# CWNE88/topdogspectrumanalyser

Hardware: AMD Instinct MI355X
Metric: PSD frames/sec at 16384-pt FFT on synthetic 20 Msps IQ (higher is better)
Workload: dtype f32; 1 GPU

## Files before the change

topdogspectrumanalyser_amd/csrc/tdsa_capi_plan.cpp:

```cpp
#include "tdsa_capi_internal.hpp"

#include <cstdarg>

using namespace tdsa;

namespace tdsa {

static thread_local char g_err[512] = "ok";

int fail(int code, const char* fmt, ...) {
  va_list ap;
  va_start(ap, fmt);
  vsnprintf(g_err, sizeof(g_err), fmt, ap);
  va_end(ap);
  return code;
}

int join_streams(tdsa_plan p) {
  if (p->aux_busy) {
    for (int i = 0; i < p->n_overlap - 1; ++i) {
      HIPCHK(hipEventRecord(p->ev_aux[i], p->aux[i]));
      HIPCHK(hipStreamWaitEvent(p->stream, p->ev_aux[i], 0));
    }
    p->aux_busy = false;
// ... 74 lines not shown
  if (!native && !chirp)
    return fail(TDSA_ERR_ARG, "nfft=%d: need a power of two in [%d, %d] or any size in [2, %d]", nfft, 1 << kMinLog2N,
                1 << kBigMaxLog2N, kChirpMaxN);
  const bool big = native && nfft > (1 << kMaxLog2N);
  if (max_frames < 1) return fail(TDSA_ERR_ARG, "max_frames=%d must be >= 1", max_frames);
  int ndev = 0;
  HIPCHK(hipGetDeviceCount(&ndev));
  if (device_id < 0 || device_id >= ndev) return fail(TDSA_ERR_ARG, "device %d of %d", device_id, ndev);
  HIPCHK(hipSetDevice(device_id));
  tdsa_plan p = new (std::nothrow) tdsa_plan_s();
  if (!p) return fail(TDSA_ERR_NOMEM, "host allocation failed");
  p->device = device_id;
  p->nfft = nfft;
  p->log2n = ilog2i(nfft);
  p->max_frames = max_frames;
  p->big = big;
  p->chirp = chirp;
  if (chirp) {
    int m = 1 << kMinLog2N;
    if (nfft > (1 << 19)) {
      p->chirp_split = (nfft + 1) / 2;
      m = 1 << kBigMaxLog2N;
    } else {
      while (m < 2 * nfft - 1) m <<= 1;
    }
    p->m_fft = m;
    p->log2m = ilog2i(m);
    p->chirp_big = p->log2m > kMaxLog2N;
    p->log2n = p->chirp_big ? kMaxLog2N : p->log2m;
  }
  const int rc_init = plan_init(p);
  if (rc_init != TDSA_OK) {
    (void)tdsa_destroy(p);
    return rc_init;
  }
  *out = p;
  return TDSA_OK;
}

static int plan_init(tdsa_plan p) {
  const int device_id = p->device, nfft = p->nfft, max_frames = p->max_frames;
  const bool big = p->big;
  hipDeviceProp_t prop;
  HIPCHK(hipGetDeviceProperties(&prop, device_id));
  p->num_cu = prop.multiProcessorCount > 0 ? prop.multiProcessorCount : 256;
  p->avg_wg_min = nfft <= 4096 ? 48 : 128;
  HIPCHK(hipStreamCreateWithFlags(&p->stream, hipStreamNonBlocking));
  HIPCHK(hipEventCreate(&p->ev0));
  HIPCHK(hipEventCreate(&p->ev1));
  HIPCHK(hipEventCreateWithFlags(&p->ev_state, hipEventDisableTiming));
  const size_t nb = size_t(nfft) * sizeof(float);
  for (int f = 0; f < 3; ++f) HIPCHK(hipMalloc(&p->d_window[f], nb));
  if (!p->big && !p->chirp && p->log2n >= 11)
    for (int f = 0; f < 3; ++f) HIPCHK(hipMalloc(&p->d_window_perm[f], nb));
  const int tw_n = p->chirp ? (p->chirp_big ? (1 << kMaxLog2N) : p->m_fft) : nfft;
  HIPCHK(hipMalloc(&p->d_hold_max, nb));
  HIPCHK(hipMalloc(&p->d_hold_min, nb));
  HIPCHK(hipMalloc(&p->d_avg, size_t(nfft) * sizeof(double)));
  HIPCHK(hipMalloc(&p->d_dc_state, sizeof(float2)));
  HIPCHK(hipMalloc(&p->d_sums, (size_t(max_frames) + 8) * sizeof(float2)));
  HIPCHK(hipMalloc(&p->d_dc_sub, size_t(max_frames) * sizeof(float2)));
  HIPCHK(hipMalloc(&p->d_tare_base, nb));
  HIPCHK(hipMalloc(&p->d_tare_acc, nb));
  HIPCHK(hipMalloc(&p->d_trace_in, nb));
  HIPCHK(hipMalloc(&p->d_trace_live, nb));
  HIPCHK(hipMemsetAsync(p->d_dc_state, 0, sizeof(float2), p->stream));
  HIPCHK(hipMemsetAsync(p->d_avg, 0, size_t(nfft) * sizeof(double), p->stream));
  TRY(upload(unit_circle(tw_n), &p->d_tw));
  if (p->chirp) TRY(chirp_plan_init(p));
  if (big) {
    HIPCHK(hipMalloc(&p->d_sum, size_t(nfft) * sizeof(double)));
    HIPCHK(hipMalloc(&p->d_lin64, size_t(nfft) * sizeof(double)));
    {
      const int n1 = nfft >> 14;
      int split = p->num_cu / n1 > 1 ? p->num_cu / n1 : 1;
      const int gmax = p->max_frames < p->big_group ? p->max_frames : p->big_group;
      if (split > gmax) split = gmax;
      HIPCHK(hipMalloc(&p->d_acc, size_t(n1) * split * (size_t(1) << 14) * sizeof(float)));
    }
    const int nrow = 1 << kMaxLog2N;
    TRY(upload(seed_table(nfft, p->log2n), &p->d_tw_seed));
    TRY(upload(unit_circle(nrow), &p->d_tw_row));
    TRY(upload(std::vector<float>(nrow, 1.0f), &p->d_ones));
  }
  TRY(reset_hold(p, true, true));
  p->mode.db_mode = TDSA_DB_MAG;
  p->mode.power_scale = 1.0f;
  p->mode.log_floor = 1e-12f;
  p->mode.avg_mode = TDSA_AVG_OFF;
  p->mode.avg_n = 1;
  p->mode.dc_alpha = 1.0f;
  p->mode.cal_offset_db = 0.0f;
  p->mode.hold_flags = 0;
  HIPCHK(hipStreamSynchronize(p->stream));
  return TDSA_OK;
}

int tdsa_destroy(tdsa_plan p) {
  if (!p) return TDSA_OK;
  (void)hipSetDevice(p->device);
  for (hipStream_t a : p->aux)
    if (a) (void)hipStreamSynchronize(a);
  if (p->stream) (void)hipStreamSynchronize(p->stream);
  free_all({p->d_window[0], p->d_window[1], p->d_window[2], p->d_window_perm[0], p->d_window_perm[1],
                  p->d_window_perm[2], p->d_tw, p->d_hold_max, p->d_hold_min,
                  p->d_avg, p->d_lin, p->d_carry, p->d_agg, p->d_agg_w, p->d_chunk_a, p->d_chunk_v, p->d_cplx, p->d_real, p->d_lin1, p->d_db1, p->d_dc_state, p->d_sums, p->d_dc_sub,
                  p->d_tare_base, p->d_tare_acc, p->d_in_stage, p->d_out_stage, p->d_trace_in,
// ... 9 lines not shown
  for (hipEvent_t e : p->prof_events) (void)hipEventDestroy(e);
  if (p->ev0) (void)hipEventDestroy(p->ev0);
  if (p->ev1) (void)hipEventDestroy(p->ev1);
  if (p->ev_state) (void)hipEventDestroy(p->ev_state);
  for (hipEvent_t e : p->ev_aux)
    if (e) (void)hipEventDestroy(e);
  for (hipStream_t a : p->aux)
    if (a) (void)hipStreamDestroy(a);
  if (p->stream) (void)hipStreamDestroy(p->stream);
  delete p;
  return TDSA_OK;
}

int tdsa_get_info(tdsa_plan p, tdsa_info* out) {
  if (!p || !out) return fail(TDSA_ERR_ARG, "null argument");
  LaunchGeom g = p->big ? spectrum_geometry(kMaxLog2N, (p->nfft >> kMaxLog2N) * (p->max_frames < p->big_group ? p->max_frames : p->big_group), p->num_cu)
                        : spectrum_geometry(p->log2n, p->max_frames, p->num_cu);
  out->nfft = p->nfft;
  out->max_frames = p->max_frames;
  out->device_id = p->device;
  out->grid = g.grid;
  out->block = g.block;
  out->frames_per_block = g.fpw;
  out->lds_bytes = int(g.lds_bytes);
  out->num_cu = p->num_cu;
  out->frames_held_max = p->held_max;
  out->frames_held_min = p->held_min;
  out->avg_count = p->avg_count;
  out->version = TDSA_VERSION;
  return TDSA_OK;
}

static void big_window_model(tdsa_plan p, const float* w, const float scale[3]) {
  bool flat = true;
  for (int i = 1; i < p->nfft && flat; ++i) flat = w[i] == w[0];
  for (int f = 0; f < 3; ++f) {
    p->big_win[f] = BigWindow{flat ? 2 : 0, p->d_window[f], w[0] * scale[f]};
  }
}

int tdsa_set_window(tdsa_plan p, const float* w_host, int n) {
  if (!p || !w_host) return fail(TDSA_ERR_ARG, "null argument");
  if (n != p->nfft) return fail(TDSA_ERR_ARG, "window length %d != nfft %d", n, p->nfft);
  HIPCHK(hipSetDevice(p->device));
  JOIN(p);
  float scale[3];
  for (int f = 0; f < 3; ++f) scale[f] = in_format_consts(f).scale;
  std::vector<float> tmp(n);
  HIPCHK(hipStreamSynchronize(p->stream));
  for (int f = 0; f < 3; ++f) {
    for (int i = 0; i < n; ++i) tmp[i] = w_host[i] * scale[f];
    HIPCHK(hipMemcpy(p->d_window[f], tmp.data(), size_t(n) * sizeof(float), hipMemcpyHostToDevice));
    if (p->d_window_perm[f]) HIPCHK(launch_window_perm(p->log2n, p->d_window[f], p->d_window_perm[f], p->stream));
  }
  if (p->big) big_window_model(p, w_host, scale);
  if (p->chirp && p->log2m >= 10) {
    std::vector<float2> aw(n);
    std::vector<double> ca(n), sa(n);
    for (int i = 0; i < n; ++i) {
      const long long q = ((long long)i * i) % (2ll * n);
      const double ang = -M_PI * double(q) / double(n);
      ca[i] = std::cos(ang);
      sa[i] = std::sin(ang);
    }
    for (int f = 0; f < 3; ++f) {
      for (int i = 0; i < n; ++i) {
        const double wv = double(w_host[i]) * double(scale[f]);
        aw[i] = float2{float(wv * ca[i]), float(wv * sa[i])};
      }
      if (!p->d_chirp_aw[f]) HIPCHK(hipMalloc(&p->d_chirp_aw[f], aw.size() * sizeof(float2)));
      HIPCHK(hipMemcpy(p->d_chirp_aw[f], aw.data(), aw.size() * sizeof(float2), hipMemcpyHostToDevice));
    }
  }
  p->window_set = true;
  return TDSA_OK;
}

int tdsa_set_mode(tdsa_plan p, const tdsa_mode* m) {
  if (!p || !m) return fail(TDSA_ERR_ARG, "null argument");
  if (m->db_mode != TDSA_DB_MAG && m->db_mode != TDSA_DB_POW) return fail(TDSA_ERR_ARG, "db_mode %d", m->db_mode);
  if (m->avg_mode < TDSA_AVG_OFF || m->avg_mode > TDSA_AVG_LIN) return fail(TDSA_ERR_ARG, "avg_mode %d", m->avg_mode);
  if (m->dc_alpha > 1.0f) return fail(TDSA_ERR_ARG, "dc_alpha %g > 1", double(m->dc_alpha));
  if (!(m->log_floor >= 0.0f)) return fail(TDSA_ERR_ARG, "log_floor must be >= 0");
  tdsa_mode nm = *m;
  if (nm.avg_n < 1) nm.avg_n = 1;
  const bool avg_changed = nm.avg_mode != p->mode.avg_mode || nm.avg_n != p->mode.avg_n;
  p->mode = nm;
  if (avg_changed) p->avg_count = 0;
  return TDSA_OK;
}

int tdsa_set_overlap(tdsa_plan p, int n_streams) {
  if (!p) return fail(TDSA_ERR_ARG, "null plan");
  if (n_streams < 1 || n_streams > tdsa_plan_s::kMaxOverlap)
    return fail(TDSA_ERR_ARG, "n_streams=%d outside [1, %d]", n_streams, tdsa_plan_s::kMaxOverlap);
  HIPCHK(hipSetDevice(p->device));
  JOIN(p);
  for (int i = 0; i < n_streams - 1; ++i) {
    if (!p->aux[i]) {
      HIPCHK(hipStreamCreateWithFlags(&p->aux[i], hipStreamNonBlocking));
      HIPCHK(hipEventCreateWithFlags(&p->ev_aux[i], hipEventDisableTiming));
    }
  }
  p->n_overlap = n_streams;
  p->rr = 0;
  return TDSA_OK;
// ... 132 lines not shown
```

topdogspectrumanalyser_amd/csrc/tdsa_kernels.hpp:

```cpp
#pragma once
#include <hip/hip_runtime.h>
#include <stddef.h>
#include <stdint.h>

#include <atomic>

namespace tdsa {

inline hipError_t ensure_dynamic_lds(const void* fn, int bytes, std::atomic<unsigned long long>& done) {
  int dev = 0;
  hipError_t e = hipGetDevice(&dev);
  if (e != hipSuccess) return e;
  const unsigned long long bit = 1ull << (dev & 63);
  if (done.load(std::memory_order_acquire) & bit) return hipSuccess;
  e = hipFuncSetAttribute(fn, hipFuncAttributeMaxDynamicSharedMemorySize, bytes);
  if (e == hipSuccess) done.fetch_or(bit, std::memory_order_release);
  return e;
}

constexpr int kMinLog2N = 6;
constexpr int kMaxLog2N = 14;

constexpr int DC_NONE = 0, DC_FRAME_MEAN = 1, DC_TRACKED = 2;

// ... 8 lines not shown
  float* out_db;
  float* out_lin;
  float2* out_cplx;
  const float2* out_mul;
  int out_mul_rows;
  int in_valid;
  int out_valid;
  const float2* dc_sub;
  float2* dc_state;
  float* part_max;
  float* part_min;
  const float* tare;
  unsigned xor_mask;
  float in_off;
  float in_scale;
  int dc_mode;
  int db_mode;
  float pscale;
  float log_floor;
  float cal_db;
  int hold_flags;
  unsigned long long* dbg;
  const float* agg_w;
  float* agg_out;
  int agg_only;
  unsigned seg_magic;
  unsigned seg_frames;
  long long seg_in_stride;
  long long seg_out_stride;
  const void* pre_raw;
  long long pre_stride;
  const float2* pre_aw;
  int pre_c64;
  unsigned pre_xor;
  float pre_off;
  int post_n;
  float post_inv_m;
  int rows_twice;
  void* stats_part;
  unsigned band_lohi;
};
constexpr int kStatsRecBytes = 16;
inline int spectrum_waves_per_frame(int log2n) { return log2n <= 10 ? 1 : (1 << log2n) / 1024; }

struct LaunchGeom {
  int grid, block, fpw;
  size_t lds_bytes;
};

LaunchGeom spectrum_geometry(int log2n, int n_frames, int num_cu);
hipError_t launch_spectrum(int log2n, int in_c64, const SpecParams& p, const LaunchGeom& g,
                           hipStream_t s);
hipError_t launch_window_perm(int log2n, const float* w, float* w_perm, hipStream_t s);

__host__ __device__ inline void spectrum_unit_range(unsigned b, unsigned n_units, unsigned grid, int& u0, int& u1) {
  const unsigned upw = n_units / grid, urem = n_units - upw * grid;
  u0 = int(b * upw + b * urem / grid);
  u1 = int((b + 1) * upw + (b + 1) * urem / grid);
}

struct AvgParams {
  const float* lin;
  int n_frames, n;
  double* state;
  int count_in;
  int mode, avg_n;
  float log_floor, cal_db;
  const float* tare;
  float* out_db;
  float* state_max;
  float* state_min;
  int first_frame_index;
  int wg_chunks;
  int wg_fold;
  int wg_fpw;
  const float* agg;
  const double* chunk_a;
  const float* chunk_v;
  const float* agg_w_local;
  int state_only;
};
constexpr int kAvgMaxWgChunks = 1024;
__host__ __device__ inline void avg_wg_range(const AvgParams& p, int b, int& f0, int& f1) {
  const int fpw = p.wg_fpw > 1 ? p.wg_fpw : 1;
  int u0, u1;
  spectrum_unit_range(unsigned(b), unsigned((p.n_frames + fpw - 1) / fpw), unsigned(p.wg_chunks), u0, u1);
  f0 = u0 * fpw < p.n_frames ? u0 * fpw : p.n_frames;
  f1 = u1 * fpw < p.n_frames ? u1 * fpw : p.n_frames;
}
hipError_t launch_avg_scan(const AvgParams& p, hipStream_t s, double* carry);
int avg_scan_chunks(int n_frames);
hipError_t launch_avg_weights(const AvgParams& p, float* w, double* chunk_a, float* chunk_v, hipStream_t s);

hipError_t launch_frame_sums(const void* in, int in_c64, unsigned xor_mask, long long frame_stride,
                             int n, int n_frames, float2* sums, hipStream_t s);
hipError_t launch_dc_track(const float2* sums, int n, int n_frames, float alpha, float in_off,
                           float in_scale, float2* dc_state, float2* dc_sub, hipStream_t s, int parts = 1);

struct TraceParams {
  const float* db_in;
  int n;
  float cal_db;
  float* tare_acc;
  int tare_collect;
  int tare_first;
  int tare_finish;
// ... 151 lines not shown
```

topdogspectrumanalyser_amd/csrc/tdsa_spectrum.hip:

```cpp
#include "tdsa_kernels.hpp"

namespace tdsa {
template <int LOG2N> hipError_t launch_size(int in_c64, const SpecParams& p, const LaunchGeom& g, hipStream_t s);
template <int LOG2N> LaunchGeom geom_size(int n_frames, int num_cu);
template <int LOG2N> hipError_t perm_size(const float* w, float* wp, hipStream_t s);

#define TDSA_FOR_SIZES(X) X(6) X(7) X(8) X(9) X(10) X(11) X(12) X(13) X(14)
#define TDSA_DECL(k)                                                                                  \
  template <> hipError_t launch_size<k>(int, const SpecParams&, const LaunchGeom&, hipStream_t);      \
  template <> LaunchGeom geom_size<k>(int, int);                                                      \
  template <> hipError_t perm_size<k>(const float*, float*, hipStream_t);
TDSA_FOR_SIZES(TDSA_DECL)

LaunchGeom spectrum_geometry(int log2n, int n_frames, int num_cu) {
  switch (log2n) {
#define TDSA_CASE(k) case k: return geom_size<k>(n_frames, num_cu);
    TDSA_FOR_SIZES(TDSA_CASE)
#undef TDSA_CASE
    default: return LaunchGeom{1, 256, 1, 0};
  }
}

hipError_t launch_window_perm(int log2n, const float* w, float* wp, hipStream_t s) {
  switch (log2n) {
#define TDSA_CASE(k) case k: return perm_size<k>(w, wp, s);
    TDSA_FOR_SIZES(TDSA_CASE)
#undef TDSA_CASE
    default: return hipErrorInvalidValue;
  }
}

hipError_t launch_spectrum(int log2n, int in_c64, const SpecParams& p, const LaunchGeom& g, hipStream_t s) {
  switch (log2n) {
#define TDSA_CASE(k) case k: return launch_size<k>(in_c64, p, g, s);
    TDSA_FOR_SIZES(TDSA_CASE)
#undef TDSA_CASE
    default: return hipErrorInvalidValue;
  }
}
}
```

topdogspectrumanalyser_amd/csrc/tdsa_spectrum_c3_inst.hip:

```cpp
#include "tdsa_spectrum_kernel.hpp"

namespace tdsa {
hipError_t launch_c3_slide(const SpecParams& p, const LaunchGeom& g, hipStream_t s) {
  return (p.hold_flags & 1) ? launch_one<14, false, 16 | 1>(p, g, s) : launch_one<14, false, 16>(p, g, s);
}
}
```

topdogspectrumanalyser_amd/csrc/tdsa_spectrum_kernel.hpp:

```cpp
#pragma once
#ifndef TDSA_DEV
#undef TDSA_TIMELINE
#undef TDSA_DYN_PRIO
#endif
#include "tdsa_fft.hpp"
#include "tdsa_kernels.hpp"
#include "tdsa_wave.hpp"

namespace tdsa {

template <int LOG2N>
struct Cfg {
  static constexpr int N = 1 << LOG2N;
  static constexpr int SG = N / 32;
  static constexpr int TPF = 2 * SG;
  static constexpr int NPASS = (N >= 2048) ? 3 : 2;
  static constexpr int A = (NPASS == 3) ? N / 1024 : N / 32;
  static constexpr int M = 32 / A;
  static constexpr int H = A / 2;
  static constexpr bool INL = (M >= 8) && (NPASS == 3);
  static constexpr int R1 = INL ? A : H;
  static constexpr int CPT = INL ? M / 2 : M;
  static constexpr int WGT = TPF > 256 ? TPF : 256;
  static constexpr int FPW = WGT / TPF;
// ... 58 lines not shown
      constexpr int i = decltype(ic)::value;
      const u32x4 q = __builtin_amdgcn_raw_buffer_load_b128(r, voff, soff + 16 * i, 0);
      dst[4 * i] = q.x; dst[4 * i + 1] = q.y; dst[4 * i + 2] = q.z; dst[4 * i + 3] = q.w;
    });
  }
}

constexpr int kRowStorePolicy = 2;
constexpr float k10Log10_2 = 3.01029995663981195214f;
constexpr float kMagExactBelow = 1e-8f;

#define TDSA_SYNC()                                                        \
  do {                                                                     \
    if constexpr (C::TPF <= 64) {                                          \
      __builtin_amdgcn_fence(__ATOMIC_RELEASE, "wavefront");               \
      __builtin_amdgcn_wave_barrier();                                     \
      __builtin_amdgcn_fence(__ATOMIC_ACQUIRE, "wavefront");               \
    } else {                                                               \
      __syncthreads();                                                     \
    }                                                                      \
  } while (0)

#ifdef TDSA_DYN_PRIO
#define TDSA_PRIO(n) __builtin_amdgcn_s_setprio(n)
#else
#define TDSA_PRIO(n) do { } while (0)
#endif

#ifdef TDSA_TIMELINE
#define TDSA_STAMP(i)                                                                              \
  do {                                                                                             \
    if (p.dbg != nullptr && blockIdx.x == 0 && (tid & 63) == 0 && unit - u0 < 8)                   \
      tl[((unit - u0) * 16 + wave) * 16 + (i)] = __builtin_amdgcn_s_memtime();                      \
  } while (0)
#else
#define TDSA_STAMP(i)
#endif

typedef float lds_v2 __attribute__((ext_vector_type(2)));
typedef __attribute__((address_space(3))) volatile lds_v2* lds_vptr;
__device__ __forceinline__ c32 lds_ld(const c32* p) {
  const lds_v2 x = *(lds_vptr)(p);
  return c32{x.x, x.y};
}
__device__ __forceinline__ void lds_st(c32* p, c32 v) { *(lds_vptr)(p) = lds_v2{v.x, v.y}; }

__device__ __forceinline__ void swap_halves(c32& a, c32& b) {
  auto rx = __builtin_amdgcn_permlane32_swap(__float_as_uint(a.x), __float_as_uint(b.x), false, false);
  auto ry = __builtin_amdgcn_permlane32_swap(__float_as_uint(a.y), __float_as_uint(b.y), false, false);
  a.x = __uint_as_float(rx[0]); b.x = __uint_as_float(rx[1]);
  a.y = __uint_as_float(ry[0]); b.y = __uint_as_float(ry[1]);
}

template <int R, int BASE, int TOT>
__device__ __forceinline__ void radix(c32 (&v)[TOT]) {
  dit<R, BASE, TOT>(v);
}

__device__ __forceinline__ void combine(c32& e, c32& o, c32 w) {
  const float x1 = fmaf(w.x, o.x, fmaf(-w.y, o.y, e.x));
  const float y1 = fmaf(w.x, o.y, fmaf(w.y, o.x, e.y));
  o = c32{fmaf(2.0f, e.x, -x1), fmaf(2.0f, e.y, -y1)};
  e = c32{x1, y1};
}
template <int U, bool EXACT = false>
__device__ __forceinline__ void combine32(c32& e, c32& o, bool odd_half) {
  const c32 orot = c32{odd_half ? o.y : o.x, odd_half ? -o.x : o.y};
  o = orot;
  bf_w<U, 32, EXACT>(e, o);
}
template <int K, int R, bool EXACT = false>
__device__ __forceinline__ void combine_const(c32& e, c32& o) {
  bf_w<K, R, EXACT>(e, o);
}

template <int LOG2N, bool IN_C64, int HOLDX, int CHIRP = 0>
__global__ void __launch_bounds__(Cfg<LOG2N>::WGT, 4) spectrum_kernel(const SpecParams p) {
  constexpr int HOLD = HOLDX & 7;
  constexpr bool STATS = (HOLDX & 8) != 0;
  constexpr bool SLIDE = (HOLDX & 16) != 0;
  using C = Cfg<LOG2N>;
  constexpr int N = C::N, SG = C::SG, A = C::A, M = C::M, H = C::H, FPW = C::FPW, NPAD = C::NPAD;
  constexpr int LH = ilog2(H);
  constexpr bool INL = C::INL;
  constexpr int R1 = C::R1;
  constexpr int LR1 = ilog2(R1);
  constexpr int CPT = C::CPT;
  constexpr int DW = (CPT >= 2) ? CPT / 2 : 1;
  constexpr int NRAW = IN_C64 ? 1 : R1 * DW;
  constexpr int ROWB = (N / A) * 2;
  constexpr int RSTEP = INL ? 1 : 2;

  extern __shared__ __attribute__((aligned(16))) unsigned char smem[];
  c32* lds = reinterpret_cast<c32*>(smem);
  c32* twm = reinterpret_cast<c32*>(smem + C::DATA_BYTES);
  double* red = reinterpret_cast<double*>(smem + C::DATA_BYTES + size_t(C::TWM) * sizeof(c32));
#ifdef TDSA_TIMELINE
  unsigned long long* tl = reinterpret_cast<unsigned long long*>(smem + C::LDS_BYTES);
#endif

  const int tid = threadIdx.x;
  const int wave = tid >> 6;
#ifdef TDSA_TIMELINE
  const unsigned long long tl_entry = __builtin_amdgcn_s_memtime();
#endif
  const int h = (tid >> 5) & 1;
  const int g = wave * 32 + (tid & 31);
  constexpr bool UNI = C::TPF >= 64;
  const int slot = (FPW == 1) ? 0 : (UNI ? __builtin_amdgcn_readfirstlane(g / SG) : g / SG);
  const int t = (FPW == 1) ? g : g - slot * SG;
  c32* buf = lds + slot * NPAD;

  const int n_units = (p.n_frames + FPW - 1) / FPW;
  const unsigned upw = unsigned(n_units) / gridDim.x, urem = unsigned(n_units) - upw * gridDim.x;
  int u0 = int(blockIdx.x * upw + blockIdx.x * urem / gridDim.x);
  int u1 = int((blockIdx.x + 1) * upw + (blockIdx.x + 1) * urem / gridDim.x);
  auto frame_of = [&](int unit) -> int {
    if constexpr (HOLD == 4 && FPW > 1) return u0 * FPW + slot * (u1 - u0) + (unit - u0);
    else return unit * FPW + slot;
  };
  constexpr unsigned SB = IN_C64 ? 8u : 2u;
  const rsrc_t win_rsrc = make_rsrc(C::WIN_LDS ? p.window : p.window_perm, N * 4u);
  float* win_lds = reinterpret_cast<float*>(smem + C::LDS_BYTES - C::WIN_BYTES);
  constexpr bool TWF_LDS = C::TWF_BYTES != 0 && HOLD == 3 && !IN_C64;
  c32* twf_tab = reinterpret_cast<c32*>(smem + C::LDS_BYTES - C::WIN_BYTES - C::TWF_BYTES);
  if constexpr (TWF_LDS) {
    if (slot == 0) {
      if (h == 0) static_for<0, 3>([&](auto ic) { constexpr int j = decltype(ic)::value; twf_tab[j * SG + t] = p.tw[t * 2 * (j + 1)]; });
      static_for<0, 4>([&](auto ic) { constexpr int a = decltype(ic)::value; twf_tab[3 * SG + a * C::TPF + h * SG + t] = p.tw[t * (8 * a + h)]; });
    }
  }
  if constexpr (C::WIN_LDS) {
    for (int i = tid; i < N; i += C::WGT) win_lds[i] = p.window[i];
    __syncthreads();
  }
  const unsigned win_voff = (unsigned(h) * SG + unsigned(t)) * 16u;
  const bool odd_half = h != 0;
  constexpr bool AGG = HOLD == 4;
  float agg[AGG ? 16 : 1];
  static_for<0, (AGG ? 16 : 1)>([&](auto ic) { agg[decltype(ic)::value] = 0.f; });
  float hmax[(HOLD & 1) ? 16 : 1], hmin[(HOLD & 2) ? 16 : 1];
  static_for<0, 16>([&](auto ic) {
    constexpr int i = decltype(ic)::value;
    if constexpr ((HOLD & 1) != 0) hmax[i] = -INFINITY;
// ... 60 lines not shown
  };
  auto out_elem_off = [&](int frame) -> long long {
    const unsigned sgm = __umulhi(unsigned(frame), p.seg_magic);
    const unsigned fi = unsigned(frame) - sgm * p.seg_frames;
    return (long long)sgm * p.seg_out_stride + (long long)fi * N;
  };

  float win[16];
  auto load_window = [&] {
    if constexpr (CHIRP != 0) {
    } else if constexpr (C::WIN_LDS) {
      static_for<0, R1>([&](auto ic) {
        constexpr int i = decltype(ic)::value;
        static_for<0, CPT>([&](auto jc) {
          constexpr int jj = decltype(jc)::value;
          if constexpr (INL) win[jj * R1 + i] = win_lds[i * (N / A) + t * M + h * CPT + jj];
          else win[jj * R1 + i] = win_lds[(2 * i + h) * (N / A) + t * M + jj];
        });
      });
    } else {
      uint32_t wq[16];
      static_for<0, 4>([&](auto qc) { constexpr int q = decltype(qc)::value; buf_load<4>(win_rsrc, win_voff, q * (2u * SG * 16u), &wq[4 * q]); });
      static_for<0, 16>([&](auto ic) { constexpr int i = decltype(ic)::value; win[i] = __uint_as_float(wq[i]); });
    }
  };
  uint32_t raw[NRAW];
  auto load_frame_raw = [&](int frame) {
    if constexpr (!IN_C64) {
      const bool act = frame < p.n_frames;
      const unsigned char* fb = static_cast<const unsigned char*>(p.in) + in_byte_off(frame);
      if constexpr (UNI) {
        const rsrc_t r = make_rsrc(fb, (FPW == 1 || act) ? N * 2u : 0u);
        static_for<0, R1>([&](auto ic) {
          constexpr int i = decltype(ic)::value;
          if constexpr (M == 1) raw[i] = unsigned(__builtin_amdgcn_raw_buffer_load_b16(r, lane_in_off, RSTEP * i * ROWB, 0));
          else buf_load<DW>(r, lane_in_off, RSTEP * i * ROWB, &raw[i * DW]);
        });
      } else {
        static_for<0, R1>([&](auto ic) {
          constexpr int i = decltype(ic)::value;
          const unsigned char* row = fb + RSTEP * i * ROWB + lane_in_off;
          if (act) {
            if constexpr (M == 1) raw[i] = *reinterpret_cast<const uint16_t*>(row);
            else load_raw<DW>(row, &raw[i * DW]);
          } else {
            static_for<0, DW>([&](auto jc) { raw[i * DW + decltype(jc)::value] = 0u; });
          }
        });
      }
    }
  };
  if (u0 < u1) load_frame_raw(frame_of(u0));
  bool slide_full = true;
  unsigned slide_sum = 0;
  typedef unsigned short slide_u16x2 __attribute__((ext_vector_type(2)));
  static_assert(!SLIDE || (LOG2N == 14 && !IN_C64 && HOLD < 2 && !STATS && CHIRP == 0 && FPW == 1 && !INL && M == 2 && NRAW == 8),
                "sliding front end: the 16384-point byte-format dB-row instantiations, hold off / max hold");
  c32 twf_lo[3], twf_hi[4];
  constexpr bool TWF_RELOAD = (CHIRP == 3 || CHIRP == 4) && (LOG2N == 11 || LOG2N == 14);
  if constexpr (!TWF_LDS && !TWF_RELOAD) {
    static_for<0, 3>([&](auto ic) { constexpr int j = decltype(ic)::value; twf_lo[j] = p.tw[t * 2 * (j + 1)]; });
    static_for<0, 4>([&](auto ic) { constexpr int a = decltype(ic)::value; twf_hi[a] = p.tw[t * (8 * a + h)]; });
  }
  if constexpr (C::NPASS == 3) {
    if (tid < C::TWM) {
      const int b = tid / A, ka = tid % A;
      twm[tid] = p.tw[ka * b * (N / (32 * A))];
    }
  }
  if constexpr (!C::WIN_LDS) load_window();

#ifdef TDSA_TIMELINE
  if (p.dbg != nullptr && blockIdx.x == 0 && (tid & 63) == 0) {
    tl[(2 * 16 + wave) * 16 + 12] = tl_entry;
    tl[(2 * 16 + wave) * 16 + 13] = __builtin_amdgcn_s_memtime();
  }
#endif
  for (int unit = u0; unit < u1; ++unit) {
    const int frame = frame_of(unit);
    const bool active = frame < p.n_frames;
    TDSA_STAMP(0);

    c32 v[16];
    float sub_re = p.in_off, sub_im = p.in_off;
    float res_re = 0.f, res_im = 0.f;
    if constexpr (IN_C64) {
      if constexpr (CHIRP == 1 || CHIRP == 3) {
        static_assert(HOLD == 0 && UNI, "fused chirp transforms: complex64 instantiation without hold, whole waves per frame");
        {
          const unsigned char* rb = static_cast<const unsigned char*>(p.pre_raw) + (long long)frame * p.pre_stride;
          const unsigned nv = active ? unsigned(p.in_valid) : 0u;
          const rsrc_t ar = make_rsrc(p.pre_aw, nv * 8u);
          float dcx = 0.f, dcy = 0.f;
          if (active && p.dc_sub != nullptr) { const float2 d = p.dc_sub[frame]; dcx = d.x; dcy = d.y; }
          const unsigned xm = p.pre_xor & 0xffffu;
          if (p.pre_c64) {
            const rsrc_t rr = make_rsrc(rb, nv * 8u);
            static_for<0, 16>([&](auto ic) {
              constexpr int idx = decltype(ic)::value;
              constexpr int jj = idx / R1, i = idx % R1;
              const u32x2 q = __builtin_amdgcn_raw_buffer_load_b64(rr, lane_in_off + jj * 8u, RSTEP * i * (N / A) * 8, 0);
              const u32x2 w = __builtin_amdgcn_raw_buffer_load_b64(ar, lane_in_off + jj * 8u, RSTEP * i * (N / A) * 8, 0);
              v[idx] = cmul(c32{__uint_as_float(q.x) - dcx, __uint_as_float(q.y) - dcy}, c32{__uint_as_float(w.x), __uint_as_float(w.y)});
            });
          } else {
            const rsrc_t rr = make_rsrc(rb, nv * 2u);
            const unsigned roff = lane_in_off >> 2;
            static_for<0, 16>([&](auto ic) {
              constexpr int idx = decltype(ic)::value;
              constexpr int jj = idx / R1, i = idx % R1;
              const unsigned u = unsigned(__builtin_amdgcn_raw_buffer_load_b16(rr, roff + jj * 2u, RSTEP * i * (N / A) * 2, 0)) ^ xm;
              const u32x2 w = __builtin_amdgcn_raw_buffer_load_b64(ar, lane_in_off + jj * 8u, RSTEP * i * (N / A) * 8, 0);
              v[idx] = cmul(c32{(float(u & 0xffu) - p.pre_off) - dcx, (float((u >> 8) & 0xffu) - p.pre_off) - dcy},
                            c32{__uint_as_float(w.x), __uint_as_float(w.y)});
            });
          }
        }
      } else {
      const unsigned char* fb = static_cast<const unsigned char*>(p.in) + in_byte_off(frame);
      static_for<0, 16>([&](auto ic) {
        constexpr int idx = decltype(ic)::value;
        constexpr int jj = idx / R1, i = idx % R1;
        const c32* row = reinterpret_cast<const c32*>(fb + RSTEP * i * (N / A) * 8 + lane_in_off);
// ... 570 lines not shown
```

topdogspectrumanalyser_amd/csrc/tdsa_spectrum_passes.inc:

```
    if constexpr (!IN_C64 && SG >= 32) {
      int* redi = reinterpret_cast<int*>(red);
      unsigned slide_ti = 0, slide_tq = 0;
      if constexpr (SLIDE) {
        if (slide_full) {
          unsigned li = 0, lq = 0;
          static_for<0, NRAW / 2>([&](auto ic) {
            constexpr int i = decltype(ic)::value;
            raw[i] ^= xm_v;
            li = __builtin_amdgcn_udot4(raw[i], 0x00010001u, li, false);
            lq = __builtin_amdgcn_udot4(raw[i], 0x01000100u, lq, false);
          });
          slide_sum = li | (lq << 16);
        }
        static_for<NRAW / 2, NRAW>([&](auto ic) {
          constexpr int i = decltype(ic)::value;
          raw[i] ^= xm_v;
          slide_ti = __builtin_amdgcn_udot4(raw[i], 0x00010001u, slide_ti, false);
          slide_tq = __builtin_amdgcn_udot4(raw[i], 0x01000100u, slide_tq, false);
        });
        const unsigned up = slide_ti | (slide_tq << 16);
        slide_ti = __builtin_amdgcn_udot2(__builtin_bit_cast(slide_u16x2, slide_sum), __builtin_bit_cast(slide_u16x2, 0x00000001u), slide_ti, false);
        slide_tq = __builtin_amdgcn_udot2(__builtin_bit_cast(slide_u16x2, slide_sum), __builtin_bit_cast(slide_u16x2, 0x00010000u), slide_tq, false);
        slide_sum = up;
      }
      if (p.dc_mode == DC_FRAME_MEAN) {
        unsigned si = 0, sq = 0;
        if constexpr (SLIDE) {
          si = slide_ti; sq = slide_tq;
        } else
        static_for<0, NRAW>([&](auto ic) {
          constexpr int i = decltype(ic)::value;
          si = __builtin_amdgcn_udot4(raw[i], 0x00010001u, si, false);
          sq = __builtin_amdgcn_udot4(raw[i], 0x01000100u, sq, false);
        });
        const int wi = dpp_wave_sum(int(si)), wq = dpp_wave_sum(int(sq));
        if constexpr (HOLD >= 3 || STATS) {
          int ws = __builtin_amdgcn_readfirstlane(wave);
          asm volatile("" : "+s"(ws));
          if ((tid & 63) == 63) *reinterpret_cast<int2*>(&redi[ws * 2]) = int2{wi, wq};
        } else {
          if ((tid & 63) == 63) *reinterpret_cast<int2*>(&redi[wave * 2]) = int2{wi, wq};
        }
      }
      TDSA_STAMP(1);
      TDSA_SYNC();
      TDSA_PRIO(3);
      TDSA_STAMP(2);
      if (p.dc_mode == DC_FRAME_MEAN) {
        const int w0 = slot * C::WPF;
        const int2 q = *reinterpret_cast<const int2*>(&redi[(w0 + (tid & (C::WPF - 1))) * 2]);
        const int ti = dpp_row_sum<C::WPF>(q.x), tq = dpp_row_sum<C::WPF>(q.y);
        sub_re = float(ti) * (1.0f / N);
        sub_im = float(tq) * (1.0f / N);
        if (p.dc_state != nullptr && frame == p.n_frames - 1 && t == 0 && h == 0)
          *p.dc_state = c32{(sub_re - p.in_off) * p.in_scale, (sub_im - p.in_off) * p.in_scale};
      } else if (p.dc_mode == DC_TRACKED && active) {
        const c32 sv = p.dc_sub[frame]; res_re = sv.x; res_im = sv.y;
      }
    } else if (!IN_C64 && p.dc_mode == DC_FRAME_MEAN) {
      unsigned si = 0, sq = 0;
      static_for<0, NRAW>([&](auto ic) {
        constexpr int i = decltype(ic)::value;
        si = __builtin_amdgcn_udot4(raw[i], 0x00010001u, si, false);
        sq = __builtin_amdgcn_udot4(raw[i], 0x01000100u, sq, false);
      });
      int ti = dpp_row_sum<SG>(int(si)), tq = dpp_row_sum<SG>(int(sq));
      ti += __shfl_xor(ti, 32);
      tq += __shfl_xor(tq, 32);
      TDSA_SYNC();
      sub_re = float(ti) * (1.0f / N);
      sub_im = float(tq) * (1.0f / N);
      if (p.dc_state != nullptr && frame == p.n_frames - 1 && t == 0 && h == 0)
        *p.dc_state = c32{(sub_re - p.in_off) * p.in_scale, (sub_im - p.in_off) * p.in_scale};
    } else if (p.dc_mode == DC_FRAME_MEAN) {
      double s_re = 0.0, s_im = 0.0;
      static_for<0, 16>([&](auto ic) {
        constexpr int i = decltype(ic)::value;
        s_re += double(v[i].x); s_im += double(v[i].y);
      });
      constexpr int W = SG < 32 ? SG : 32;
      s_re = wave_sum<W>(s_re); s_im = wave_sum<W>(s_im);
      s_re += __shfl_xor(s_re, 32); s_im += __shfl_xor(s_im, 32);
      if constexpr (SG > 32) {
        if constexpr (HOLD >= 3 || STATS) {
          int ws = __builtin_amdgcn_readfirstlane(wave);
          asm volatile("" : "+s"(ws));
          if ((tid & 63) == 0) { red[ws * 2] = s_re; red[ws * 2 + 1] = s_im; }
        } else {
          if ((tid & 63) == 0) { red[wave * 2] = s_re; red[wave * 2 + 1] = s_im; }
        }
      }
      TDSA_SYNC();
      if constexpr (SG > 32) {
        const int w0 = slot * C::WPF;
        s_re = 0.0; s_im = 0.0;
#pragma unroll
        for (int i = 0; i < C::WPF; ++i) { s_re += red[(w0 + i) * 2]; s_im += red[(w0 + i) * 2 + 1]; }
      }
      sub_re = float(s_re * (1.0 / N));
      sub_im = float(s_im * (1.0 / N));
      if (p.dc_state != nullptr && frame == p.n_frames - 1 && t == 0 && h == 0)
        *p.dc_state = c32{(sub_re - p.in_off) * p.in_scale, (sub_im - p.in_off) * p.in_scale};
    } else {
      TDSA_SYNC();
      if (p.dc_mode == DC_TRACKED && active) {
        const c32 s = p.dc_sub[frame];
        if constexpr (IN_C64) { sub_re = s.x; sub_im = s.y; }
        else { res_re = s.x; res_im = s.y; }
      }
    }
    sub_re = in_vgpr(sub_re);
    sub_im = in_vgpr(sub_im);
    if constexpr (C::WIN_LDS) load_window();

    constexpr bool FUSE_WIN = R1 >= 2 && CHIRP == 0;
    auto put = [&](auto ic, float xr, float xi) {
      constexpr int idx = decltype(ic)::value;
      if constexpr (FUSE_WIN || CHIRP != 0) v[idx] = c32{xr, xi};
      else v[idx] = c32{xr * win[idx], xi * win[idx]};
    };
    if constexpr (IN_C64) {
      static_for<0, 16>([&](auto ic) {
        constexpr int i = decltype(ic)::value;
        put(ic, v[i].x - sub_re, v[i].y - sub_im);
      });
    } else if constexpr (M == 1) {
      static_for<0, 16>([&](auto ic) {
        constexpr int i = decltype(ic)::value;
        const uint32_t u = raw[i];
        put(ic, float(u & 0xffu) - sub_re, float((u >> 8) & 0xffu) - sub_im);
      });
    } else if constexpr (FUSE_WIN) {
      auto pair = [&](auto ac, float exr, float exi, float oxr, float oxi) {
        constexpr int a = decltype(ac)::value, b = a + R1 / 2;
        const float er = (exr - sub_re) * win[a], ei = (exi - sub_im) * win[a];
        const float orr = oxr - sub_re, oi = oxi - sub_im;
        v[a] = c32{fmaf(orr, win[b], er), fmaf(oi, win[b], ei)};
        v[b] = c32{fmaf(-orr, win[b], er), fmaf(-oi, win[b], ei)};
      };
      static_for<0, R1 / 2>([&](auto ic) {
        constexpr int i = decltype(ic)::value;
        static_for<0, DW>([&](auto dc) {
          constexpr int d = decltype(dc)::value;
          const uint32_t ue = raw[i * DW + d], uo = raw[(i + R1 / 2) * DW + d];
          pair(std::integral_constant<int, (2 * d) * R1 + i>{}, float(ue & 0xffu), float((ue >> 8) & 0xffu),
               float(uo & 0xffu), float((uo >> 8) & 0xffu));
          pair(std::integral_constant<int, (2 * d + 1) * R1 + i>{}, float((ue >> 16) & 0xffu), float(ue >> 24),
               float((uo >> 16) & 0xffu), float(uo >> 24));
        });
      });
    } else {
      static_for<0, R1>([&](auto ic) {
        constexpr int i = decltype(ic)::value;
        static_for<0, DW>([&](auto dc) {
          constexpr int d = decltype(dc)::value;
          const uint32_t u = raw[i * DW + d];
          constexpr int i0 = (2 * d) * R1 + i, i1 = (2 * d + 1) * R1 + i;
          put(std::integral_constant<int, i0>{}, float(u & 0xffu) - sub_re, float((u >> 8) & 0xffu) - sub_im);
          put(std::integral_constant<int, i1>{}, float((u >> 16) & 0xffu) - sub_re, float(u >> 24) - sub_im);
        });
      });
    }
    if constexpr (FUSE_WIN && (IN_C64 || M == 1)) {
      static_for<0, CPT>([&](auto jc) {
        constexpr int jj = decltype(jc)::value;
        static_for<0, R1 / 2>([&](auto ic) {
          constexpr int a = jj * R1 + decltype(ic)::value, b = a + R1 / 2;
          const float er = v[a].x * win[a], ei = v[a].y * win[a];
          const float orr = v[b].x, oi = v[b].y;
          v[a] = c32{fmaf(orr, win[b], er), fmaf(oi, win[b], ei)};
          v[b] = c32{fmaf(-orr, win[b], er), fmaf(-oi, win[b], ei)};
        });
      });
    }
    if constexpr (!IN_C64) {
      if (p.dc_mode == DC_TRACKED) {
        if constexpr (FUSE_WIN) {
          static_for<0, CPT>([&](auto jc) {
            constexpr int jj = decltype(jc)::value;
            static_for<0, R1 / 2>([&](auto ic) {
              constexpr int a = jj * R1 + decltype(ic)::value, b = a + R1 / 2;
              const float ws = win[a] + win[b], wd = win[a] - win[b];
              v[a] = c32{fmaf(-res_re, ws, v[a].x), fmaf(-res_im, ws, v[a].y)};
              v[b] = c32{fmaf(-res_re, wd, v[b].x), fmaf(-res_im, wd, v[b].y)};
            });
          });
        } else {
          static_for<0, 16>([&](auto ic) {
            constexpr int i = decltype(ic)::value;
            v[i] = c32{fmaf(-res_re, win[i], v[i].x), fmaf(-res_im, win[i], v[i].y)};
          });
        }
      }
    }
    TDSA_STAMP(3);
    if constexpr (SLIDE) {
      if (unit + 1 < u1) {
        const int nf = frame_of(unit + 1);
        slide_full = p.seg_magic != 0u && unsigned(nf) - __umulhi(unsigned(nf), p.seg_magic) * p.seg_frames == 0u;
        if (slide_full) {
          load_frame_raw(nf);
        } else {
          const rsrc_t r = make_rsrc(static_cast<const unsigned char*>(p.in) + in_byte_off(nf), N * 2u);
          static_for<0, NRAW / 2>([&](auto ic) {
            constexpr int i = decltype(ic)::value;
            raw[i] = raw[i + NRAW / 2];
            raw[i + NRAW / 2] = __builtin_amdgcn_raw_buffer_load_b32(r, lane_in_off, RSTEP * (i + NRAW / 2) * ROWB, 0);
          });
        }
      }
    } else
    if (unit + 1 < u1) load_frame_raw(frame_of(unit + 1));
    TDSA_PRIO(2);

    if constexpr (FUSE_WIN) static_for<0, CPT>([&](auto jc) { dit_rest<R1, decltype(jc)::value * R1, 16>(v); });
    else static_for<0, CPT>([&](auto jc) { radix<R1, decltype(jc)::value * R1, 16>(v); });
    if constexpr (INL) {
      static_for<0, 16>([&](auto ec) {
        constexpr int e = decltype(ec)::value;
        constexpr int g = e / A, k = e % A;
        lds_st(&buf[wr1_base + e], v[g * A + bitrev(k, LR1)]);
      });
    } else {
    TDSA_PRIO(1);
    static_for<0, 8>([&](auto uc) {
      constexpr int u = decltype(uc)::value;
      if constexpr (u == 4) TDSA_PRIO(0);
      constexpr int jj0 = u / H, k0 = u % H, jj1 = (u + 8) / H, k1 = (u + 8) % H;
      constexpr int re = jj0 * H + bitrev(k0, LH), ro = jj1 * H + bitrev(k1, LH);
      swap_halves(v[re], v[ro]);
      if constexpr (A == 32) combine32<u>(v[re], v[ro], odd_half);
      else combine_const<k0, A>(v[re], v[ro]);
      constexpr int li = jj0 * A + k0;
      { lds_st(&buf[wr1_base + li], v[re]); lds_st(&buf[wr1_base + li + H], v[ro]); }
    });
    }
    TDSA_STAMP(4);
    TDSA_SYNC();
    TDSA_PRIO(3);
    TDSA_STAMP(5);

    if constexpr (C::NPASS == 3) {
      static_for<0, 16>([&](auto ic) {
        constexpr int i = decltype(ic)::value;
        v[i] = lds_ld(&buf[rdA + i * 2 * rd_stride]);
      });
      int tw_o = h * A + ka_mid;
      asm volatile("" : "+v"(tw_o));
      static_for<0, 2>([&](auto bc) {
        constexpr int b0 = decltype(bc)::value * 4;
        c32 tw8[8];
        static_for<0, 8>([&](auto ic) {
          constexpr int q = decltype(ic)::value;
          constexpr int i = b0 + (q & 3) + 8 * (q >> 2);
          tw8[q] = twm[tw_o + i * 2 * A];
        });
        __builtin_amdgcn_sched_barrier(0);
        static_for<0, 4>([&](auto ic) {
          constexpr int q = decltype(ic)::value;
          bf_tw(v[b0 + q], v[b0 + q + 8], tw8[q], tw8[q + 4]);
        });
        __builtin_amdgcn_sched_barrier(0);
      });
      TDSA_STAMP(6);
      TDSA_PRIO(2);
      dit_rest<16, 0, 16>(v);
      TDSA_PRIO(1);
      static_for<0, 8>([&](auto uc) {
        constexpr int u = decltype(uc)::value;
        if constexpr (u == 4) TDSA_PRIO(0);
        constexpr int re = bitrev(u, 4), ro = bitrev(u + 8, 4);
        swap_halves(v[re], v[ro]);
        combine32<u>(v[re], v[ro], odd_half);
        {
          lds_st(&buf[wrM + u * rd_stride], v[re]);
          lds_st(&buf[wrM + (u + 16) * rd_stride], v[ro]);
        }
      });
      TDSA_STAMP(7);
      TDSA_SYNC();
      TDSA_PRIO(3);
      TDSA_STAMP(8);
      static_for<0, 16>([&](auto ic) {
        constexpr int i = decltype(ic)::value;
        v[i] = lds_ld(&buf[rd3A + 2 * i * A + ((2 * i * A) >> 5)]);
      });
    } else {
      static_for<0, 16>([&](auto ic) {
// ... 34 lines not shown
```

Baseline: 34.79 million frames/s.

## Regroup raw rows in-lane for the 16K slide kernel with a dedicated window table

For the 16384-point slide path, raw input rows are regrouped inside each lane with byte permutes and permlane32 swaps. The first FFT stage then becomes a radix-2·R1 butterfly computed entirely in registers, replacing the cross-lane swap-halves/combine step before the LDS store. A second permuted window table matching the new in-lane element order is built at window-set time and passed to the kernel. This aims to cut cross-lane shuffle and combine work per frame, at the cost of extra perm instructions, added register pressure and a doubled window buffer.

Result: faster. 35.23 million frames/s, median of 6 (+1.3%).

```diff
diff --git a/topdogspectrumanalyser_amd/csrc/tdsa_c3_inlane.hpp b/topdogspectrumanalyser_amd/csrc/tdsa_c3_inlane.hpp
--- /dev/null
+++ b/topdogspectrumanalyser_amd/csrc/tdsa_c3_inlane.hpp
@@ -0,0 +1,15 @@
+#pragma once
+
+namespace tdsa {
+
+constexpr int kC3InlaneN = 16384;
+constexpr int kC3InlaneRows = 16;
+constexpr int kC3InlaneSG = 512;
+
+constexpr int c3_inlane_window_index(int slot) {
+  const int entry = slot & 3, th = (slot >> 2) % (2 * kC3InlaneSG), quarter = (slot >> 2) / (2 * kC3InlaneSG);
+  const int h = th / kC3InlaneSG, t = th % kC3InlaneSG, a = 4 * quarter + entry;
+  return a * (kC3InlaneN / kC3InlaneRows) + 2 * t + h;
+}
+
+}
diff --git a/topdogspectrumanalyser_amd/csrc/tdsa_capi_plan.cpp b/topdogspectrumanalyser_amd/csrc/tdsa_capi_plan.cpp
--- a/topdogspectrumanalyser_amd/csrc/tdsa_capi_plan.cpp
+++ b/topdogspectrumanalyser_amd/csrc/tdsa_capi_plan.cpp
@@ -150,7 +150,8 @@
   const size_t nb = size_t(nfft) * sizeof(float);
   for (int f = 0; f < 3; ++f) HIPCHK(hipMalloc(&p->d_window[f], nb));
   if (!p->big && !p->chirp && p->log2n >= 11)
-    for (int f = 0; f < 3; ++f) HIPCHK(hipMalloc(&p->d_window_perm[f], nb));
+    for (int f = 0; f < 3; ++f)
+      HIPCHK(hipMalloc(&p->d_window_perm[f], c3_window_tables(p->log2n, f == TDSA_IN_C64) ? 2 * nb : nb));
   const int tw_n = p->chirp ? (p->chirp_big ? (1 << kMaxLog2N) : p->m_fft) : nfft;
   HIPCHK(hipMalloc(&p->d_hold_max, nb));
   HIPCHK(hipMalloc(&p->d_hold_min, nb));
@@ -266,6 +267,8 @@
     for (int i = 0; i < n; ++i) tmp[i] = w_host[i] * scale[f];
     HIPCHK(hipMemcpy(p->d_window[f], tmp.data(), size_t(n) * sizeof(float), hipMemcpyHostToDevice));
     if (p->d_window_perm[f]) HIPCHK(launch_window_perm(p->log2n, p->d_window[f], p->d_window_perm[f], p->stream));
+    if (p->d_window_perm[f] && c3_window_tables(p->log2n, f == TDSA_IN_C64))
+      HIPCHK(launch_window_perm_c3_inlane(p->d_window[f], p->d_window_perm[f] + n, p->stream));
   }
   if (p->big) big_window_model(p, w_host, scale);
   if (p->chirp && p->log2m >= 10) {
diff --git a/topdogspectrumanalyser_amd/csrc/tdsa_kernels.hpp b/topdogspectrumanalyser_amd/csrc/tdsa_kernels.hpp
--- a/topdogspectrumanalyser_amd/csrc/tdsa_kernels.hpp
+++ b/topdogspectrumanalyser_amd/csrc/tdsa_kernels.hpp
@@ -84,6 +84,8 @@
 hipError_t launch_spectrum(int log2n, int in_c64, const SpecParams& p, const LaunchGeom& g,
                            hipStream_t s);
 hipError_t launch_window_perm(int log2n, const float* w, float* w_perm, hipStream_t s);
+inline bool c3_window_tables(int log2n, int in_c64) { return log2n == 14 && !in_c64; }
+hipError_t launch_window_perm_c3_inlane(const float* w, float* w_perm_c3, hipStream_t s);
 
 __host__ __device__ inline void spectrum_unit_range(unsigned b, unsigned n_units, unsigned grid, int& u0, int& u1) {
   const unsigned upw = n_units / grid, urem = n_units - upw * grid;
diff --git a/topdogspectrumanalyser_amd/csrc/tdsa_spectrum.hip b/topdogspectrumanalyser_amd/csrc/tdsa_spectrum.hip
--- a/topdogspectrumanalyser_amd/csrc/tdsa_spectrum.hip
+++ b/topdogspectrumanalyser_amd/csrc/tdsa_spectrum.hip
@@ -1,3 +1,4 @@
+#include "tdsa_c3_inlane.hpp"
 #include "tdsa_kernels.hpp"
 
 namespace tdsa {
@@ -30,6 +31,15 @@
   }
 }
 
+__global__ void __launch_bounds__(256) window_perm_c3_inlane_kernel(const float* w, float* wp) {
+  const int slot = blockIdx.x * 256 + threadIdx.x;
+  if (slot < kC3InlaneN) wp[slot] = w[c3_inlane_window_index(slot)];
+}
+hipError_t launch_window_perm_c3_inlane(const float* w, float* wp, hipStream_t s) {
+  hipLaunchKernelGGL(window_perm_c3_inlane_kernel, dim3(kC3InlaneN / 256), dim3(256), 0, s, w, wp);
+  return hipGetLastError();
+}
+
 hipError_t launch_spectrum(int log2n, int in_c64, const SpecParams& p, const LaunchGeom& g, hipStream_t s) {
   switch (log2n) {
 #define TDSA_CASE(k) case k: return launch_size<k>(in_c64, p, g, s);
diff --git a/topdogspectrumanalyser_amd/csrc/tdsa_spectrum_c3_inst.hip b/topdogspectrumanalyser_amd/csrc/tdsa_spectrum_c3_inst.hip
--- a/topdogspectrumanalyser_amd/csrc/tdsa_spectrum_c3_inst.hip
+++ b/topdogspectrumanalyser_amd/csrc/tdsa_spectrum_c3_inst.hip
@@ -1,7 +1,12 @@
+#include "tdsa_c3_inlane.hpp"
 #include "tdsa_spectrum_kernel.hpp"
 
 namespace tdsa {
+static_assert(kC3InlaneN == Cfg<14>::N && kC3InlaneRows == Cfg<14>::A && kC3InlaneSG == Cfg<14>::SG, "tdsa_c3_inlane.hpp describes Cfg<14>");
+
 hipError_t launch_c3_slide(const SpecParams& p, const LaunchGeom& g, hipStream_t s) {
-  return (p.hold_flags & 1) ? launch_one<14, false, 16 | 1>(p, g, s) : launch_one<14, false, 16>(p, g, s);
+  SpecParams q = p;
+  q.window_perm = p.window_perm + Cfg<14>::N;
+  return (q.hold_flags & 1) ? launch_one<14, false, 16 | 1>(q, g, s) : launch_one<14, false, 16>(q, g, s);
 }
 }
diff --git a/topdogspectrumanalyser_amd/csrc/tdsa_spectrum_kernel.hpp b/topdogspectrumanalyser_amd/csrc/tdsa_spectrum_kernel.hpp
--- a/topdogspectrumanalyser_amd/csrc/tdsa_spectrum_kernel.hpp
+++ b/topdogspectrumanalyser_amd/csrc/tdsa_spectrum_kernel.hpp
@@ -134,6 +134,13 @@
   a.y = __uint_as_float(ry[0]); b.y = __uint_as_float(ry[1]);
 }
 
+__device__ __forceinline__ void regroup_rows(uint32_t& a, uint32_t& b) {
+  const uint32_t lo = __builtin_amdgcn_perm(b, a, 0x05040100u);
+  const uint32_t hi = __builtin_amdgcn_perm(b, a, 0x07060302u);
+  auto r = __builtin_amdgcn_permlane32_swap(lo, hi, false, false);
+  a = r[0]; b = r[1];
+}
+
 template <int R, int BASE, int TOT>
 __device__ __forceinline__ void radix(c32 (&v)[TOT]) {
   dit<R, BASE, TOT>(v);
@@ -172,6 +179,8 @@
   constexpr int NRAW = IN_C64 ? 1 : R1 * DW;
   constexpr int ROWB = (N / A) * 2;
   constexpr int RSTEP = INL ? 1 : 2;
+  constexpr int R1L = SLIDE ? 2 * R1 : R1;
+  constexpr int CPTL = SLIDE ? CPT / 2 : CPT;
 
   extern __shared__ __attribute__((aligned(16))) unsigned char smem[];
   c32* lds = reinterpret_cast<c32*>(smem);
diff --git a/topdogspectrumanalyser_amd/csrc/tdsa_spectrum_passes.inc b/topdogspectrumanalyser_amd/csrc/tdsa_spectrum_passes.inc
--- a/topdogspectrumanalyser_amd/csrc/tdsa_spectrum_passes.inc
+++ b/topdogspectrumanalyser_amd/csrc/tdsa_spectrum_passes.inc
@@ -4,6 +4,7 @@
       if constexpr (SLIDE) {
         if (slide_full) {
           unsigned li = 0, lq = 0;
+          static_for<0, NRAW / 4>([&](auto ic) { regroup_rows(raw[2 * decltype(ic)::value], raw[2 * decltype(ic)::value + 1]); });
           static_for<0, NRAW / 2>([&](auto ic) {
             constexpr int i = decltype(ic)::value;
             raw[i] ^= xm_v;
@@ -12,6 +13,7 @@
           });
           slide_sum = li | (lq << 16);
         }
+        static_for<NRAW / 4, NRAW / 2>([&](auto ic) { regroup_rows(raw[2 * decltype(ic)::value], raw[2 * decltype(ic)::value + 1]); });
         static_for<NRAW / 2, NRAW>([&](auto ic) {
           constexpr int i = decltype(ic)::value;
           raw[i] ^= xm_v;
@@ -132,12 +134,22 @@
       });
     } else if constexpr (FUSE_WIN) {
       auto pair = [&](auto ac, float exr, float exi, float oxr, float oxi) {
-        constexpr int a = decltype(ac)::value, b = a + R1 / 2;
+        constexpr int a = decltype(ac)::value, b = a + R1L / 2;
         const float er = (exr - sub_re) * win[a], ei = (exi - sub_im) * win[a];
         const float orr = oxr - sub_re, oi = oxi - sub_im;
         v[a] = c32{fmaf(orr, win[b], er), fmaf(oi, win[b], ei)};
         v[b] = c32{fmaf(-orr, win[b], er), fmaf(-oi, win[b], ei)};
       };
+      if constexpr (SLIDE) {
+        static_for<0, NRAW / 2>([&](auto kc) {
+          constexpr int k = decltype(kc)::value, a = (k >> 1) * 4 + (k & 1);
+          const uint32_t ue = raw[k], uo = raw[k + NRAW / 2];
+          pair(std::integral_constant<int, a>{}, float(ue & 0xffu), float((ue >> 8) & 0xffu),
+               float(uo & 0xffu), float((uo >> 8) & 0xffu));
+          pair(std::integral_constant<int, a + 2>{}, float((ue >> 16) & 0xffu), float(ue >> 24),
+               float((uo >> 16) & 0xffu), float(uo >> 24));
+        });
+      } else
       static_for<0, R1 / 2>([&](auto ic) {
         constexpr int i = decltype(ic)::value;
         static_for<0, DW>([&](auto dc) {
@@ -176,10 +188,10 @@
     if constexpr (!IN_C64) {
       if (p.dc_mode == DC_TRACKED) {
         if constexpr (FUSE_WIN) {
-          static_for<0, CPT>([&](auto jc) {
+          static_for<0, CPTL>([&](auto jc) {
             constexpr int jj = decltype(jc)::value;
-            static_for<0, R1 / 2>([&](auto ic) {
-              constexpr int a = jj * R1 + decltype(ic)::value, b = a + R1 / 2;
+            static_for<0, R1L / 2>([&](auto ic) {
+              constexpr int a = jj * R1L + decltype(ic)::value, b = a + R1L / 2;
               const float ws = win[a] + win[b], wd = win[a] - win[b];
               v[a] = c32{fmaf(-res_re, ws, v[a].x), fmaf(-res_im, ws, v[a].y)};
               v[b] = c32{fmaf(-res_re, wd, v[b].x), fmaf(-res_im, wd, v[b].y)};
@@ -213,6 +225,15 @@
     if (unit + 1 < u1) load_frame_raw(frame_of(unit + 1));
     TDSA_PRIO(2);
 
+    if constexpr (SLIDE) {
+      dit_s<R1, 0, 2, 16, true>(v);
+      dit_s<R1, 1, 2, 16, true>(v);
+      static_for<0, R1>([&](auto kc) {
+        constexpr int k = decltype(kc)::value, slot = 2 * bitrev(k, LR1);
+        bf_w<k, R1L>(v[slot], v[slot + 1]);
+        { lds_st(&buf[wr1_base + k], v[slot]); lds_st(&buf[wr1_base + k + R1], v[slot + 1]); }
+      });
+    } else {
     if constexpr (FUSE_WIN) static_for<0, CPT>([&](auto jc) { dit_rest<R1, decltype(jc)::value * R1, 16>(v); });
     else static_for<0, CPT>([&](auto jc) { radix<R1, decltype(jc)::value * R1, 16>(v); });
     if constexpr (INL) {
@@ -234,6 +255,7 @@
       constexpr int li = jj0 * A + k0;
       { lds_st(&buf[wr1_base + li], v[re]); lds_st(&buf[wr1_base + li + H], v[ro]); }
     });
+    }
     }
     TDSA_STAMP(4);
     TDSA_SYNC();
```

## Compute sliding DC mean via i8 MFMA and LDS atomics instead of dot/DPP reductions

Applied to the files above, without the earlier changes.

In the sliding front end, per-lane I/Q byte sums are computed with an i8 MFMA against a lane-dependent selector vector instead of per-register udot4 chains. The wave-level DPP reductions are replaced by workgroup-scope atomic adds into double-buffered LDS slots, which are reset for the next frame after the barrier. This aims to cut VALU and cross-lane reduction work on the frame-mean path, at the cost of MFMA latency, LDS atomic contention, an extra init barrier and subtle dependence on lane/selector layout.

Result: no change. 34.46 million frames/s before, 34.71 million frames/s after (median of 6 runs) (+0.7%).

```diff
diff --git a/topdogspectrumanalyser_amd/csrc/tdsa_spectrum_kernel.hpp b/topdogspectrumanalyser_amd/csrc/tdsa_spectrum_kernel.hpp
--- a/topdogspectrumanalyser_amd/csrc/tdsa_spectrum_kernel.hpp
+++ b/topdogspectrumanalyser_amd/csrc/tdsa_spectrum_kernel.hpp
@@ -338,8 +338,8 @@
   };
   if (u0 < u1) load_frame_raw(frame_of(u0));
   bool slide_full = true;
-  unsigned slide_sum = 0;
-  typedef unsigned short slide_u16x2 __attribute__((ext_vector_type(2)));
+  int slide_sum = 0;
+  typedef int slide_i32x4 __attribute__((ext_vector_type(4)));
   static_assert(!SLIDE || (LOG2N == 14 && !IN_C64 && HOLD < 2 && !STATS && CHIRP == 0 && FPW == 1 && !INL && M == 2 && NRAW == 8),
                 "sliding front end: the 16384-point byte-format dB-row instantiations, hold off / max hold");
   c32 twf_lo[3], twf_hi[4];
@@ -355,6 +355,10 @@
     }
   }
   if constexpr (!C::WIN_LDS) load_window();
+  if constexpr (SLIDE) {
+    if (tid < 4) reinterpret_cast<int*>(red)[tid] = 128 * N;
+    __syncthreads();
+  }
 
 #ifdef TDSA_TIMELINE
   if (p.dbg != nullptr && blockIdx.x == 0 && (tid & 63) == 0) {
diff --git a/topdogspectrumanalyser_amd/csrc/tdsa_spectrum_passes.inc b/topdogspectrumanalyser_amd/csrc/tdsa_spectrum_passes.inc
--- a/topdogspectrumanalyser_amd/csrc/tdsa_spectrum_passes.inc
+++ b/topdogspectrumanalyser_amd/csrc/tdsa_spectrum_passes.inc
@@ -1,33 +1,40 @@
     if constexpr (!IN_C64 && SG >= 32) {
       int* redi = reinterpret_cast<int*>(red);
-      unsigned slide_ti = 0, slide_tq = 0;
+      int slide_tot = 0;
+      unsigned slide_t8 = 0;
       if constexpr (SLIDE) {
-        if (slide_full) {
-          unsigned li = 0, lq = 0;
-          static_for<0, NRAW / 2>([&](auto ic) {
-            constexpr int i = decltype(ic)::value;
-            raw[i] ^= xm_v;
-            li = __builtin_amdgcn_udot4(raw[i], 0x00010001u, li, false);
-            lq = __builtin_amdgcn_udot4(raw[i], 0x01000100u, lq, false);
-          });
-          slide_sum = li | (lq << 16);
-        }
-        static_for<NRAW / 2, NRAW>([&](auto ic) {
-          constexpr int i = decltype(ic)::value;
-          raw[i] ^= xm_v;
-          slide_ti = __builtin_amdgcn_udot4(raw[i], 0x00010001u, slide_ti, false);
-          slide_tq = __builtin_amdgcn_udot4(raw[i], 0x01000100u, slide_tq, false);
-        });
-        const unsigned up = slide_ti | (slide_tq << 16);
-        slide_ti = __builtin_amdgcn_udot2(__builtin_bit_cast(slide_u16x2, slide_sum), __builtin_bit_cast(slide_u16x2, 0x00000001u), slide_ti, false);
-        slide_tq = __builtin_amdgcn_udot2(__builtin_bit_cast(slide_u16x2, slide_sum), __builtin_bit_cast(slide_u16x2, 0x00010000u), slide_tq, false);
+        asm volatile("v_lshlrev_b32 %0, 1, %1" : "=v"(slide_t8) : "v"(out_voff));
+        const int sel1 = int(__builtin_amdgcn_alignbit(0x00010001u, 0x00010001u, slide_t8));
+        const slide_i32x4 sel = {sel1, sel1, sel1, sel1};
+        const unsigned sx = p.xor_mask ^ 0x80808080u;
+        auto half_sum = [&](auto bc) -> int {
+          constexpr int b = decltype(bc)::value;
+          slide_i32x4 d;
+          if (sx == 0u) {
+            d = __builtin_amdgcn_mfma_i32_16x16x64_i8(slide_i32x4{int(raw[b]), int(raw[b + 1]), int(raw[b + 2]), int(raw[b + 3])}, sel,
+                                                      slide_i32x4{0, 0, 0, 0}, 0, 0, 0);
+          } else {
+            d = __builtin_amdgcn_mfma_i32_16x16x64_i8(slide_i32x4{int(raw[b] ^ sx), int(raw[b + 1] ^ sx), int(raw[b + 2] ^ sx), int(raw[b + 3] ^ sx)}, sel,
+                                                      slide_i32x4{0, 0, 0, 0}, 0, 0, 0);
+          }
+          static_for<b, b + 4>([&](auto ic) { raw[decltype(ic)::value] ^= xm_v; });
+          return (d.x + d.y) + (d.z + d.w);
+        };
+        if (slide_full) slide_sum = half_sum(std::integral_constant<int, 0>{});
+        const int up = half_sum(std::integral_constant<int, NRAW / 2>{});
+        slide_tot = slide_sum + up;
         slide_sum = up;
       }
+      const int slide_slot = SLIDE ? (unit & 1) : 0;
+      if constexpr (SLIDE) {
+        if (p.dc_mode == DC_FRAME_MEAN) {
+          if ((tid & 14) == 14)
+            __hip_atomic_fetch_add(reinterpret_cast<int*>(reinterpret_cast<char*>(&redi[slide_slot]) + (slide_t8 & 8u)), slide_tot, __ATOMIC_RELAXED,
+                                   __HIP_MEMORY_SCOPE_WORKGROUP);
+        }
+      } else
       if (p.dc_mode == DC_FRAME_MEAN) {
         unsigned si = 0, sq = 0;
-        if constexpr (SLIDE) {
-          si = slide_ti; sq = slide_tq;
-        } else
         static_for<0, NRAW>([&](auto ic) {
           constexpr int i = decltype(ic)::value;
           si = __builtin_amdgcn_udot4(raw[i], 0x00010001u, si, false);
@@ -46,6 +53,22 @@
       TDSA_SYNC();
       TDSA_PRIO(3);
       TDSA_STAMP(2);
+      if constexpr (SLIDE) {
+        if (p.dc_mode == DC_FRAME_MEAN) {
+          const int2 q = int2{redi[slide_slot], redi[slide_slot + 2]};
+          if (tid == 0) {
+            int z = 128 * N;
+            asm volatile("" : "+v"(z));
+            redi[slide_slot ^ 1] = z; redi[(slide_slot ^ 1) + 2] = z;
+          }
+          sub_re = float(q.x) * (1.0f / N);
+          sub_im = float(q.y) * (1.0f / N);
+          if (p.dc_state != nullptr && frame == p.n_frames - 1 && t == 0 && h == 0)
+            *p.dc_state = c32{(sub_re - p.in_off) * p.in_scale, (sub_im - p.in_off) * p.in_scale};
+        } else if (p.dc_mode == DC_TRACKED && active) {
+          const c32 sv = p.dc_sub[frame]; res_re = sv.x; res_im = sv.y;
+        }
+      } else
       if (p.dc_mode == DC_FRAME_MEAN) {
         const int w0 = slot * C::WPF;
         const int2 q = *reinterpret_cast<const int2*>(&redi[(w0 + (tid & (C::WPF - 1))) * 2]);
```
